# shubhamchandak94/HARC

Hardware: AMD Instinct MI355X
Metric: Mreads/s reorder+encode, 100 bp (higher is better)
Workload: dtype u64 (2-bit packed bases, XOR+popcount)

## Files before the change

### harc_amd/csrc/internal.h

```cpp
#pragma once
#include <hip/hip_runtime.h>
#include <stdint.h>
#include <stdio.h>
#include <string.h>
#include <map>
#include <string>
#include <utility>
#include <vector>
#include "../../include/harc_amd.h"

#define HARC_NONE 0xFFFFFFFFu
#define HARC_MAXW 8
#define HARC_MAXW3 12
#define HARC_MAXK (1u << 20)
#define HARC_LOOK_CHUNKS 16
#ifndef HARC_NSUGG
#define HARC_NSUGG 8
#endif

void harc_set_error(const char *fmt, ...);

#define HIP_TRY(expr)                                                                                          \
    do {                                                                                                       \
        hipError_t _e = (expr);                                                                                \
// ... 96 lines not shown
    harc_amd_counters C;
    uint64_t digest[4] = { 0, 0, 0, 0 }; bool have_digest = false;

    char *feed_ring = nullptr; size_t feed_ring_bytes = 0;

    void *d_tmp = nullptr; size_t tmp_bytes = 0;
};

struct HarcComm {
    int world = 1, rank = 0;
    virtual ~HarcComm() {}
    virtual int allgather_u64(harc_amd_ctx *c, const uint64_t *in, int n, uint64_t *out) = 0;
    virtual int alltoallv(harc_amd_ctx *c, int narr, const void *const *send, const size_t *const *soff, const size_t *const *sbytes,
                          void *const *recv, const size_t *const *roff, const size_t *const *rbytes) = 0;
    virtual int allreduce_min_u64(harc_amd_ctx *c, unsigned long long *d_buf, size_t n) = 0;
    virtual int wait(harc_amd_ctx *c, const char *what) = 0;
    virtual const char *name() const = 0;
};
int harc_in_reserve(harc_amd_ctx *c, harc_amd_ctx::InBuf *b, size_t bytes);
void harc_reset_shard(harc_amd_ctx *c);
void harc_drop_results(harc_amd_ctx *c);

int harc_dev_alloc(harc_amd_ctx *c, void **p, size_t bytes);
void harc_dev_free(harc_amd_ctx *c, void *p);
template <class T> static inline int dalloc(harc_amd_ctx *c, T **p, size_t n) { return harc_dev_alloc(c, (void **)p, n * sizeof(T) + 16); }
int harc_tmp_reserve(harc_amd_ctx *c, size_t bytes);
int harc_raw_alloc(harc_amd_ctx *c, void **p, size_t bytes);
void harc_raw_free(harc_amd_ctx *c, void *p);
typedef unsigned long long harc_mark_t;
harc_mark_t harc_pool_mark(harc_amd_ctx *c);
void harc_pool_release(harc_amd_ctx *c, harc_mark_t m);
struct PoolScope {
    harc_amd_ctx *c; harc_mark_t mk; bool armed = true;
    explicit PoolScope(harc_amd_ctx *c_) : c(c_), mk(harc_pool_mark(c_)) {}
    PoolScope(const PoolScope &) = delete;
    PoolScope &operator=(const PoolScope &) = delete;
    ~PoolScope() { if (armed) harc_pool_release(c, mk); }
    void keep() { armed = false; }
    void release_now() { if (armed) { harc_pool_release(c, mk); armed = false; } }
};

int prim_sort_pairs_u64_u32(harc_amd_ctx *c, const uint64_t *kin, uint64_t *kout, const uint32_t *vin, uint32_t *vout, size_t n, unsigned end_bit);
#define BL_TILE_WORDS 16384u
#define BL_PART_BITS 20
#define harc_bitmap_tiles(nwords) ((uint32_t)(((uint64_t)(nwords) + BL_TILE_WORDS - 1) / BL_TILE_WORDS))
#define harc_bitmap_item(w, b0, b1) (((uint64_t)((((uint32_t)(w) % BL_TILE_WORDS) << 10) | ((uint32_t)(b0) << 5) | (uint32_t)(b1)) << BL_PART_BITS) | (uint64_t)((uint32_t)(w) / BL_TILE_WORDS))
int harc_bitmap_from_items(harc_amd_ctx *c, const uint64_t *items, uint64_t *tmp, size_t n, uint64_t nwords, uint32_t *bitmap);
int prim_sort_keys_u64(harc_amd_ctx *c, const uint64_t *kin, uint64_t *kout, size_t n, unsigned end_bit);
int prim_excl_scan_u32(harc_amd_ctx *c, const uint32_t *in, uint32_t *out, size_t n);
int prim_excl_scan_u32_to_u64(harc_amd_ctx *c, const uint32_t *in, uint64_t *out, size_t n);
int prim_excl_scan_u8_to_u64(harc_amd_ctx *c, const uint8_t *in, uint64_t *out, size_t n);
int prim_incl_scan_u64(harc_amd_ctx *c, const uint64_t *in, uint64_t *out, size_t n);
int prim_incl_max_u32(harc_amd_ctx *c, const uint32_t *in, uint32_t *out, size_t n);
int prim_incl_max_u64(harc_amd_ctx *c, const uint64_t *in, uint64_t *out, size_t n);

int s1_pack_ascii(harc_amd_ctx *c, const char *d_ascii, uint32_t n, uint32_t stride, uint64_t *d_out);
int s1_pack3_ascii(harc_amd_ctx *c, const char *d_ascii, uint32_t n, uint32_t stride, uint64_t *d_out);
int s1_unpack_to_ascii(harc_amd_ctx *c, const uint64_t *d_reads, uint32_t n, char *d_out);
int s1_bucket_reads(harc_amd_ctx *c, const uint64_t *d_packed, uint32_t n, uint32_t nb, uint32_t *d_out);
int s1_partition_reads(harc_amd_ctx *c, const uint64_t *d_packed, uint32_t n, uint32_t nb, uint64_t *d_out, unsigned long long *d_counts);
int shard_partition(harc_amd_ctx *c, const uint64_t *d_words, uint32_t n, int nwords, bool three_bit, uint32_t nb, uint32_t gid0,
                    uint64_t *d_out, uint32_t *d_gid_out, unsigned long long *d_counts);
int shard_map_ids(harc_amd_ctx *c, uint32_t *d_v, uint64_t n, const uint32_t *d_map, uint32_t nmap, unsigned int *d_err);
int stage1_run(harc_amd_ctx *c);
int stage1_make_oriented(harc_amd_ctx *c, uint32_t i0 = 0, uint32_t i1 = 0xFFFFFFFFu);
int s1_orient(harc_amd_ctx *c, const uint64_t *reads, const uint32_t *order, const uint8_t *rc, uint32_t m, uint64_t *out);
int harc_dict_alloc(harc_amd_ctx *c, DictDev *d, uint32_t n, uint64_t cap_like);
int harc_dict_build(harc_amd_ctx *c, DictDev *d, uint64_t *keys, uint32_t *ids, uint32_t n, unsigned kbits);
void harc_dict_free(harc_amd_ctx *c, DictDev *d);
int stage2_run(harc_amd_ctx *c);
int pack_order_run(harc_amd_ctx *c);

static inline std::vector<uint8_t> &out_buf(harc_amd_ctx *c, int id, int shard) { harc_amd_ctx::OutBuf &o = c->out[std::make_pair(id, shard)]; o.ptr = nullptr; o.len = 0; return o.own; }
static inline void out_slice(harc_amd_ctx *c, int id, int shard, const void *p, size_t n) { harc_amd_ctx::OutBuf &o = c->out[std::make_pair(id, shard)]; o.own.clear(); o.ptr = (const uint8_t *)p; o.len = n; }
int harc_host_alloc(harc_amd_ctx *c, void **p, size_t bytes);
void harc_host_reset(harc_amd_ctx *c);
int harc_d2h(harc_amd_ctx *c, std::vector<uint8_t> &dst, const void *d_src, size_t bytes);

int build_line_index(harc_amd_ctx *c, const char *d_txt, uint64_t nbytes, const uint64_t **nls_out, uint64_t *total_lines_out);

struct BgzfCand { uint64_t off; uint32_t bsize, hdr, isize, crc; };
struct BgzfMember { uint64_t cdata, text; uint32_t clen, isize, crc, hdr; };
struct BgzfPlan { std::vector<BgzfMember> m; uint64_t text = 0, next = 0; };
int harc_bgzf_plan(harc_amd_ctx *c, const uint8_t *d_in, uint64_t n, uint64_t start, uint64_t own_end, uint64_t base_off, BgzfPlan *plan);
int harc_bgzf_run(harc_amd_ctx *c, const uint8_t *d_in, const BgzfPlan &plan, uint64_t base_off, char *d_out);

struct BgzfOutStats { uint64_t text = 0, bytes = 0, members = 0, stored = 0; double seconds = 0; };
int harc_bgzf_deflate(harc_amd_ctx *c, const char *d_text, uint64_t n_bytes, int32_t flags, uint8_t *d_out, uint64_t out_capacity, uint64_t *n_out, BgzfOutStats *st);
```

### harc_amd/csrc/prims.hip

```cpp
#include "devutil.h"
#include <rocprim/rocprim.hpp>

int harc_tmp_reserve(harc_amd_ctx *c, size_t bytes)
{
    if (bytes <= c->tmp_bytes) return HARC_AMD_OK;
    if (c->d_tmp) harc_raw_free(c, c->d_tmp);
    c->d_tmp = nullptr; c->tmp_bytes = 0;
    size_t want = bytes + (bytes >> 3) + 4096;
    RC_TRY(harc_raw_alloc(c, &c->d_tmp, want));
    c->tmp_bytes = want;
    return HARC_AMD_OK;
}

#define PRIM_CALL(call_with_tmp)                                \
    do {                                                        \
        size_t bytes = 0; void *tmp = nullptr;                  \
        HIP_TRY(call_with_tmp);                                 \
        RC_TRY(harc_tmp_reserve(c, bytes));                     \
        tmp = c->d_tmp; bytes = c->tmp_bytes;                   \
        HIP_TRY(call_with_tmp);                                 \
    } while (0)

int prim_sort_pairs_u64_u32(harc_amd_ctx *c, const uint64_t *kin, uint64_t *kout, const uint32_t *vin, uint32_t *vout, size_t n, unsigned end_bit)
{
    if (n == 0) return HARC_AMD_OK;
    if (end_bit > 64) end_bit = 64;
    PRIM_CALL(rocprim::radix_sort_pairs(tmp, bytes, kin, kout, vin, vout, n, 0u, end_bit, c->stream));
    return HARC_AMD_OK;
}

int prim_sort_keys_u64(harc_amd_ctx *c, const uint64_t *kin, uint64_t *kout, size_t n, unsigned end_bit)
{
    if (n == 0) return HARC_AMD_OK;
    if (end_bit > 64) end_bit = 64;
    if (end_bit < 1) end_bit = 1;
    PRIM_CALL(rocprim::radix_sort_keys(tmp, bytes, kin, kout, n, 0u, end_bit, c->stream));
    return HARC_AMD_OK;
}

int prim_excl_scan_u32(harc_amd_ctx *c, const uint32_t *in, uint32_t *out, size_t n)
{
    if (n == 0) return HARC_AMD_OK;
    PRIM_CALL(rocprim::exclusive_scan(tmp, bytes, in, out, 0u, n, rocprim::plus<uint32_t>(), c->stream));
    return HARC_AMD_OK;
}

struct u32_to_u64 { __host__ __device__ uint64_t operator()(uint32_t x) const { return (uint64_t)x; } };
struct u8_to_u64 { __host__ __device__ uint64_t operator()(uint8_t x) const { return (uint64_t)x; } };

int prim_excl_scan_u32_to_u64(harc_amd_ctx *c, const uint32_t *in, uint64_t *out, size_t n)
{
    if (n == 0) return HARC_AMD_OK;
    auto it = rocprim::make_transform_iterator(in, u32_to_u64());
    PRIM_CALL(rocprim::exclusive_scan(tmp, bytes, it, out, (uint64_t)0, n, rocprim::plus<uint64_t>(), c->stream));
    return HARC_AMD_OK;
}

int prim_excl_scan_u8_to_u64(harc_amd_ctx *c, const uint8_t *in, uint64_t *out, size_t n)
{
    if (n == 0) return HARC_AMD_OK;
    auto it = rocprim::make_transform_iterator(in, u8_to_u64());
    PRIM_CALL(rocprim::exclusive_scan(tmp, bytes, it, out, (uint64_t)0, n, rocprim::plus<uint64_t>(), c->stream));
    return HARC_AMD_OK;
}

int prim_incl_scan_u64(harc_amd_ctx *c, const uint64_t *in, uint64_t *out, size_t n)
{
    if (n == 0) return HARC_AMD_OK;
    PRIM_CALL(rocprim::inclusive_scan(tmp, bytes, in, out, n, rocprim::plus<uint64_t>(), c->stream));
    return HARC_AMD_OK;
}

int prim_incl_max_u32(harc_amd_ctx *c, const uint32_t *in, uint32_t *out, size_t n)
{
    if (n == 0) return HARC_AMD_OK;
    PRIM_CALL(rocprim::inclusive_scan(tmp, bytes, in, out, n, rocprim::maximum<uint32_t>(), c->stream));
    return HARC_AMD_OK;
}

int prim_incl_max_u64(harc_amd_ctx *c, const uint64_t *in, uint64_t *out, size_t n)
{
    if (n == 0) return HARC_AMD_OK;
    PRIM_CALL(rocprim::inclusive_scan(tmp, bytes, in, out, n, rocprim::maximum<uint64_t>(), c->stream));
    return HARC_AMD_OK;
}

__global__ void k_selftest_grid(uint64_t n, unsigned long long *out)
{
    const uint64_t i = harc_gid();
    unsigned long long one = i < n ? 1ULL : 0ULL, idx = i < n ? (unsigned long long)i : 0ULL;
    for (int o = 32; o > 0; o >>= 1) { one += __shfl_xor(one, o, 64); idx += __shfl_xor(idx, o, 64); }
    if ((threadIdx.x & 63) == 0 && one) { atomicAdd(&out[0], one); atomicAdd(&out[1], idx); }
}
__global__ void k_selftest_grid32(uint32_t n, unsigned long long *out)
{
    const uint32_t i = harc_gid32();
    unsigned long long one = i < n ? 1ULL : 0ULL, idx = i < n ? (unsigned long long)i : 0ULL;
    for (int o = 32; o > 0; o >>= 1) { one += __shfl_xor(one, o, 64); idx += __shfl_xor(idx, o, 64); }
    if ((threadIdx.x & 63) == 0 && one) { atomicAdd(&out[0], one); atomicAdd(&out[1], idx); }
}
__global__ void k_selftest_fold(uint64_t n, unsigned long long *out)
{
    const uint64_t wave = harc_bid() * 4 + (threadIdx.x >> 6);
    const int lane = threadIdx.x & 63;
    const uint64_t i = wave * 16 + (uint64_t)(lane >> 2);
    const bool mine = i < n && (lane & 3) == 0;
    unsigned long long one = mine ? 1ULL : 0ULL, idx = mine ? (unsigned long long)i : 0ULL;
    for (int o = 32; o > 0; o >>= 1) { one += __shfl_xor(one, o, 64); idx += __shfl_xor(idx, o, 64); }
    if (lane == 0 && one) { atomicAdd(&out[0], one); atomicAdd(&out[1], idx); }
}
extern "C" int harc_amd_selftest_launch(harc_amd_ctx *c, uint64_t n, uint64_t *visited, uint64_t *index_sum)
{
    if (!c || !visited || !index_sum) return HARC_AMD_EINVAL;
    HIP_TRY(hipSetDevice(c->P.device));
    unsigned long long *d = nullptr, h[6] = { 0, 0, 0, 0, 0, 0 };
    HIP_TRY(hipMalloc((void **)&d, sizeof h));
    const bool n32 = n <= 0xFFFFFFFFull;
    hipError_t e = hipMemsetAsync(d, 0, sizeof h, c->stream);
    if (e == hipSuccess) { hipLaunchKernelGGL(k_selftest_grid, harc_grid256(n), dim3(256), 0, c->stream, n, d); e = hipGetLastError(); }
    if (e == hipSuccess && n32) { hipLaunchKernelGGL(k_selftest_grid32, harc_grid256(n), dim3(256), 0, c->stream, (uint32_t)n, d + 2); e = hipGetLastError(); }
    if (e == hipSuccess) { hipLaunchKernelGGL(k_selftest_fold, harc_fold256((n + 63) / 64), dim3(256), 0, c->stream, n, d + 4); e = hipGetLastError(); }
    if (e == hipSuccess) e = hipMemcpyAsync(h, d, sizeof h, hipMemcpyDeviceToHost, c->stream);
    if (e == hipSuccess) e = hipStreamSynchronize(c->stream);
    (void)hipFree(d);
    if (e != hipSuccess) { harc_set_error("harc_amd_selftest_launch: %s", hipGetErrorString(e)); return HARC_AMD_ENODEVICE; }
    int k = 0;
    if (n32 && (h[2] != h[0] || h[3] != h[1])) k = 2;
    else if (h[4] != h[0] || h[5] != h[1]) k = 4;
    if (k) harc_set_error("harc_amd_selftest_launch: %s visited %llu items (index sum %llx), the thread-per-item grid %llu (%llx)", k == 2 ? "harc_gid32" : "harc_fold256 / harc_bid", h[k], h[k + 1], h[0], h[1]);
    *visited = h[k]; *index_sum = h[k + 1];
    return k ? HARC_AMD_EINTERNAL : HARC_AMD_OK;
}
```

### harc_amd/csrc/stage1.hip

```cpp
#include "devutil.h"
#include <stdlib.h>
#include <type_traits>

struct S1Args {
    int L, maxmatch, thresh, maxsearch, Lp;
    int ds[2], de[2], kbits[2];
    uint32_t N, K;
    const uint64_t *reads;
    HashSlot *slots[2];
    uint64_t cap[2];
    const uint32_t *ids[2];
    int firstmax;
    const uint32_t *bloom[2]; uint32_t bloom_lines; int bloom_nwin[2]; uint32_t bloom_mmask;
    const uint2 *largetab;
    uint64_t *mirror;
    unsigned long long *claimed;
    uint32_t *bid;
    ChainHdr *hdr;
    uint4 *cnt;
    uint2 *steps;
    uint8_t *need;
    uint32_t *seedbuf;
    uint32_t *needrank;
    uint32_t *rmeta;
    uint32_t own_mod, own_rem;
    uint32_t reseed_stress;
    uint32_t reseed_win;
    unsigned int *reseed_g;
    uint2 *cst2;
    uint32_t *bo;
    uint32_t *sugg;
    int S;
    int nsugg_per_seed;
    int nsugg_stride;
    uint2 *slog;
    uint2 *pg_rec;
    uint2 *pg_hdr;
    uint32_t *pg_cur;
    unsigned int *pg_count;
    long long *cursor;
    unsigned long long *coopcnt;
    unsigned long long *stats;
    const uint16_t *probe_tab;
    const uint32_t *lds_tab;
    int nprobe;
    int budget;
    int stepcap;
    int weedmin;
    int lazy;
    uint4 *cstat_coop;
    uint2 *csteps;
    uint4 *cstat;
    const uint2 *succ;
    unsigned long long *dbg;
// ... 156 lines not shown
    return HARC_AMD_OK;
}

template <int W> __global__ void k_keygen2(const uint64_t *reads, uint32_t n, int off0, int nbits0, int off1, int nbits1, uint64_t *keys0, uint64_t *keys1, uint32_t *ids)
{
    const uint32_t i = harc_gid32();
    if (i >= n) return;
    uint64_t r[W];
#pragma unroll
    for (int w = 0; w < W; w++) r[w] = reads[(size_t)i * W + w];
    {
        const int wi = off0 >> 6, sh = off0 & 63;
        const uint64_t lo = sel0<W>(r, wi), hi = sel0<W>(r, wi + 1);
        uint64_t v = sh ? ((lo >> sh) | (hi << (64 - sh))) : lo;
        if (nbits0 < 64) v &= ((uint64_t)1 << nbits0) - 1;
        keys0[i] = v;
    }
    {
        const int wi = off1 >> 6, sh = off1 & 63;
        const uint64_t lo = sel0<W>(r, wi), hi = sel0<W>(r, wi + 1);
        uint64_t v = sh ? ((lo >> sh) | (hi << (64 - sh))) : lo;
        if (nbits1 < 64) v &= ((uint64_t)1 << nbits1) - 1;
        keys1[i] = v;
    }
    ids[i] = i;
}
__global__ void k_large_sizes(const unsigned long long *list, uint32_t nlist, HashSlot *s0, HashSlot *s1, uint32_t *sz)
{
    const uint32_t b = harc_gid32();
    if (b >= nlist) return;
    const unsigned long long e = list[b];
    const HashSlot *slot = ((e & 1) ? s1 : s0) + (e >> 1);
    sz[b] = slot->count & SLOT_CNT_MASK;
}
template <int W> __global__ __launch_bounds__(64) void k_large_fill(const unsigned long long *list, uint32_t nlist, HashSlot *s0, HashSlot *s1, const uint32_t *ids0, const uint32_t *ids1,
                                                                   const uint64_t *moff, const uint64_t *reads, uint2 *largetab, uint64_t *mirror)
{
    const uint32_t b = blockIdx.y * gridDim.x + blockIdx.x;
    if (b >= nlist) return;
    const int lane = threadIdx.x;
    const unsigned long long e = list[b];
    const int l = (int)(e & 1);
    HashSlot *slot = (l ? s1 : s0) + (e >> 1);
    const uint32_t st = slot->start, cnt = slot->count & SLOT_CNT_MASK;
    const uint32_t *ids = (l ? ids1 : ids0) + st;
    const uint64_t m0 = moff[b];
    for (uint32_t k = lane; k < cnt; k += 64) {
        const uint32_t rid = ids[k];
#pragma unroll
        for (int w = 0; w < W; w++) mirror[(m0 + k) * W + w] = reads[(size_t)rid * W + w];
    }
    if (lane == 0) { largetab[b] = make_uint2(st, (uint32_t)m0); slot->start = b; }
}
__global__ void k_mark_heads(const uint64_t *skeys, uint32_t n, uint32_t *head)
{
    const uint32_t i = harc_gid32();
    if (i >= n) return;
    head[i] = (i == 0 || skeys[i] != skeys[i - 1]) ? 1u : 0u;
}
__global__ void k_bin_starts(const uint32_t *head, const uint32_t *binidx, uint32_t n, uint32_t *binstart, uint32_t *nbins, const uint64_t *skeys, uint64_t cap, uint64_t *v)
{
    const uint32_t i = harc_gid32();
    if (i >= n) return;
    if (head[i]) { const uint32_t b = binidx[i]; binstart[b] = i; v[b] = bucket_slot(skeys[i], cap) + (uint64_t)n - (uint64_t)b; }
    if (i == n - 1) *nbins = binidx[i] + head[i];
}
#define HARC_LARGEBIN 16u
#define HARC_STEP_CAP 12
#define HARC_BO_FREE 1u
#define HARC_BO_CAP 3u
#define HARC_SCAN_BUDGET 12
#define MIXED_MAX (1u << 20)
#define MIXED_BUDGET 200000u
__device__ __forceinline__ uint64_t rotl64(uint64_t x, unsigned r) { r &= 63u; return r ? (x << r) | (x >> (64u - r)) : x; }
__global__ void k_mixed_find(const uint64_t *rk, uint32_t n, unsigned sbits, uint64_t *sk, uint32_t *list, unsigned int *meta)
{
    const uint32_t i = harc_gid32();
    if (i >= n) return;
    const int shift = (int)(64u - sbits);
    const uint64_t b = rotl64(rk[i], 64u - sbits);
    sk[i] = b;
    if (i == 0) return;
    const uint64_t a = rotl64(rk[i - 1], 64u - sbits);
    if (a != b && (a >> shift) == (b >> shift)) { const unsigned int at = atomicAdd(&meta[0], 1u); if (at < MIXED_MAX) list[at] = i; else meta[1] = 1u; }
}
__global__ void k_mixed_own(const uint64_t *sk, int shift, uint32_t *list, unsigned int *meta)
{
    const uint32_t t = harc_gid32();
    const unsigned int nl = meta[0] < MIXED_MAX ? meta[0] : MIXED_MAX;
    if (t >= nl || meta[1]) return;
    const uint32_t i = list[t];
    const uint64_t top = sk[i] >> shift;
    for (uint32_t h = i; h > 0 && (sk[h - 1] >> shift) == top;) {
        h--;
        if (h > 0 && sk[h] != sk[h - 1] && (sk[h - 1] >> shift) == top) { list[t] = HARC_NONE; return; }
        if (i - h > MIXED_BUDGET) { meta[1] = 1u; return; }
    }
}
__global__ void k_mixed_fix(uint64_t *sk, uint32_t *ids, uint32_t n, int shift, const uint32_t *list, unsigned int *meta)
{
    const uint32_t t = harc_gid32();
    const unsigned int nl = meta[0] < MIXED_MAX ? meta[0] : MIXED_MAX;
    if (t >= nl || meta[1]) return;
    const uint32_t i = list[t];
    if (i == HARC_NONE) return;
    const uint64_t top = sk[i] >> shift;
    uint32_t h = i;
    while (h > 0 && (sk[h - 1] >> shift) == top) h--;
    uint32_t e = i + 1;
    while (e < n && (sk[e] >> shift) == top) { e++; if (e - h > MIXED_BUDGET) { meta[1] = 1u; return; } }
    uint32_t moves = 0;
    for (uint32_t x = h + 1; x < e; x++) {
        const uint64_t kx = sk[x]; const uint32_t vx = ids[x];
        uint32_t y = x;
        while (y > h && sk[y - 1] > kx) { sk[y] = sk[y - 1]; ids[y] = ids[y - 1]; y--; if (++moves > MIXED_BUDGET) { meta[1] = 1u; return; } }
        if (y != x) { sk[y] = kx; ids[y] = vx; }
    }
}
__global__ void k_scramble_keys(uint64_t *keys, uint32_t n, unsigned rot)
{
    const uint32_t i = harc_gid32();
    if (i < n) keys[i] = rotl64(key_scramble(keys[i]), rot);
}
__global__ void k_rotate_keys(uint64_t *keys, uint32_t n, unsigned rot)
{
    const uint32_t i = harc_gid32();
    if (i < n) keys[i] = rotl64(keys[i], rot);
}
#ifndef TP_SPAN
#define TP_SPAN 1280u
#endif
__global__ __launch_bounds__(256) void k_table_place(const uint64_t *skeys, const uint32_t *sids, const uint32_t *binstart, uint32_t nbins, uint32_t n, const uint64_t *q,
                              HashSlot *slots, uint64_t cap, uint32_t bigthresh,
                              unsigned long long *large_list, unsigned int *large_n, uint32_t large_max, uint32_t large_tag, uint32_t *nbins_p, int pass, uint32_t first_block, int fill)
{
    __shared__ uint4 tile[TP_SPAN];
    if (blockIdx.x < first_block) return;
    const uint32_t i = harc_gid32();
    const bool have = i < nbins;
    auto slot_of = [&](uint32_t k) -> uint64_t { return q[k] - (uint64_t)n + (uint64_t)k; };
    const uint32_t b0 = blockIdx.x * blockDim.x, b1 = b0 + blockDim.x < nbins ? b0 + blockDim.x : nbins;
    bool tiled = false; uint64_t lo = 0, hi = 0;
    if (pass == 0 && fill && b0 < nbins) {
        lo = b0 ? slot_of(b0 - 1) + 1 : 0;
        const uint64_t last = slot_of(b1 - 1);
        if (lo < cap) {
            hi = (last >= cap || b1 == nbins || slot_of(b1) >= cap) ? cap : last + 1;
            tiled = hi - lo <= TP_SPAN;
        }
    }
    if (tiled) {
        const uint4 z = make_uint4(0u, 0u, 0u, 0u);
        for (uint32_t j = threadIdx.x; j < (uint32_t)(hi - lo); j += blockDim.x) tile[j] = z;
        __syncthreads();
    }
    uint64_t sl = have ? slot_of(i) : 0;
    bool mine = have;
    if (mine && pass == 0 && sl >= cap && blockIdx.x + 64 < gridDim.x) { atomicAdd(nbins_p + 1, 1u); mine = false; }
    if (mine && (pass == 1) != (sl >= cap)) mine = false;
    if (mine) {
        const uint32_t st = binstart[i];
        const uint64_t key = skeys[st];
        uint32_t ovf = 0;
        if (pass == 0 && (sl & 3) == 0 && (uint64_t)i + 4 < (uint64_t)nbins) {
            const uint64_t s3 = slot_of(i + 3);
            if (s3 == sl + 3 && (bucket_slot(skeys[binstart[i + 4]], cap) >> 2) <= (sl >> 2)) ovf = SLOT_OVF;
        }
        if (pass == 0 && fill && !tiled) {
            const uint4 z = make_uint4(0u, 0u, 0u, 0u);
            for (uint64_t x = i ? slot_of(i - 1) + 1 : 0; x < sl; x++) *reinterpret_cast<uint4 *>(&slots[x]) = z;
            if (i + 1 == nbins || slot_of(i + 1) >= cap)
                for (uint64_t x = sl + 1; x < cap; x++) *reinterpret_cast<uint4 *>(&slots[x]) = z;
        }
        const uint32_t en = (i + 1 < nbins) ? binstart[i + 1] : n;
        const uint32_t cnt = en - st;
        if (cnt > SLOT_CNT_MASK) atomicAdd(nbins_p + 1, 1u);
        else {
            const unsigned long long meta = cnt == 1 ? ((unsigned long long)sids[st] | ((unsigned long long)(1u | SLOT_EMB) << 32))
                                                     : ((unsigned long long)st | ((unsigned long long)((cnt & SLOT_CNT_MASK) | ((bigthresh && cnt > bigthresh) ? SLOT_BIG : 0u)) << 32));
            if (pass == 1) {
                for (uint64_t bb = bucket_slot(key, cap) >> 2; bb < (cap >> 2); bb++) atomicOr(&slots[4 * bb].count, SLOT_OVF);
                sl = 0;
                for (;;) {
                    unsigned long long *mp = reinterpret_cast<unsigned long long *>(&slots[sl]) + 1;
                    if (atomicCAS(mp, 0ULL, meta) == 0ULL) break;
                    if ((sl & 3) == 3) atomicOr(&slots[sl - 3].count, SLOT_OVF);
                    if (++sl == cap) sl = 0;
                }
                slots[sl].key = key;
            } else {
                uint4 w; w.x = (uint32_t)key; w.y = (uint32_t)(key >> 32); w.z = (uint32_t)meta; w.w = (uint32_t)(meta >> 32) | ovf;
                if (tiled) tile[sl - lo] = w; else *reinterpret_cast<uint4 *>(&slots[sl]) = w;
            }
            if (large_list && cnt > HARC_LARGEBIN) {
                const unsigned int at = atomicAdd(large_n, 1u);
                if (at < large_max) large_list[at] = ((unsigned long long)sl << 1) | large_tag;
            }
        }
    }
    if (tiled) {
        __syncthreads();
        for (uint32_t j = threadIdx.x; j < (uint32_t)(hi - lo); j += blockDim.x) *reinterpret_cast<uint4 *>(&slots[lo + j]) = tile[j];
    }
}

__global__ void k_s1_bloom_keys(const uint64_t *keys, uint32_t n, uint32_t nlines, int nwin, uint32_t mmask, uint64_t *pk)
{
    const uint32_t i = harc_gid32();
    if (i >= n) return;
    uint32_t w, m;
    bloom_pos(keys[i], key_scramble(keys[i]), nlines, nwin, mmask, &w, &m);
    const uint32_t b0 = (uint32_t)__ffs((int)m) - 1u, b1 = 31u - (uint32_t)__clz((int)m);
    pk[i] = harc_bitmap_item(w, b0, b1);
}
__global__ __launch_bounds__(256) void k_s1_bloom_tile(const uint64_t *pk, uint32_t n, uint64_t nwords, uint32_t *bloom)
{
    __shared__ uint32_t tile[BL_TILE_WORDS];
    __shared__ uint32_t bounds[2];
    const uint32_t part = blockIdx.x;
// ... 1924 lines not shown
}
__global__ __launch_bounds__(256) void k_pages_out(const uint2 *pg_rec, const uint2 *pg_hdr, uint32_t npages, const uint32_t *n_main, const uint32_t *base_main,
                                                   uint32_t *order, uint8_t *flag, uint8_t *pos, uint8_t *rc)
{
    const uint32_t p = blockIdx.x * 4 + (threadIdx.x >> 6), lane = threadIdx.x & 63;
    if (p >= npages) return;
    const uint2 hd = pg_hdr[p];
    const uint32_t nm = n_main[hd.x], first = hd.y * 64u;
    if (first + lane >= nm) return;
    const uint2 r = pg_rec[(size_t)p * 64 + lane];
    const size_t at = (size_t)base_main[hd.x] + first + lane;
    order[at] = r.x; pos[at] = (uint8_t)(r.y & 0xFF);
    flag[at] = (r.y >> 8) & 1 ? '1' : '0'; rc[at] = (r.y >> 9) & 1 ? 'r' : 'd';
}
template <int W> __global__ void k_orient(const uint64_t *reads, const uint32_t *order, const uint8_t *rc, uint32_t m, int L, uint64_t *out)
{
    constexpr int RPW = 64 / W;
    const int lane = threadIdx.x & 63, rl = lane / W, w = lane % W;
    const uint64_t wave = harc_gid() >> 6;
    const uint64_t i64 = wave * RPW + (uint64_t)rl;
    const uint32_t i = (uint32_t)i64;
    const bool on = rl < RPW && i64 < m;
    uint64_t mine = 0; bool rev = false;
    if (on) {
        const uint32_t rid = order[i];
        mine = reads[(size_t)rid * W + w];
        rev = rc != nullptr && rc[i] == 'r';
    }
    uint64_t r[W], o[W];
#pragma unroll
    for (int k = 0; k < W; k++) r[k] = shfl_u64(mine, rl * W + k);
    if (!on) return;
    uint64_t ow = mine;
    if (rev) { rc_words<W>(r, L, o); ow = sel0<W>(o, w); }
    out[(size_t)i * W + w] = ow;
}

int harc_dict_alloc(harc_amd_ctx *c, DictDev *d, uint32_t n, uint64_t cap_like)
{
    d->cap = 0; d->slots = nullptr; d->ids = nullptr; d->d_nbins = nullptr;
    if (n == 0) return HARC_AMD_OK;
    if (cap_like) d->cap = cap_like;
    else {
        unsigned long long m = 4;
        size_t fr = 0, tot = 0;
        if (hipMemGetInfo(&fr, &tot) == hipSuccess) { fr += c->pool_total; while (m > 2 && ((double)m * n * sizeof(HashSlot) > 0.2 * (double)fr || (double)m * n * sizeof(HashSlot) > 0.15 * (double)tot)) m--; }
        if (c->P.table_slots_per_read >= 2 && c->P.table_slots_per_read <= 4) m = (unsigned long long)c->P.table_slots_per_read;
        if (const char *e = getenv("HARC_AMD_CAPMULT")) m = strtoull(e, nullptr, 10);
        d->cap = (((m < 2 ? 2 : m) * n + 4) + 3) & ~3ull;
    }
    RC_TRY(dalloc(c, &d->slots, d->cap)); RC_TRY(dalloc(c, &d->ids, n)); RC_TRY(dalloc(c, &d->d_nbins, 2));
    return HARC_AMD_OK;
}
int harc_dict_build(harc_amd_ctx *c, DictDev *d, uint64_t *keys, uint32_t *ids, uint32_t n, unsigned kbits)
{
    (void)kbits;
    if (n == 0) return HARC_AMD_OK;
    PoolScope scope(c);
    uint64_t *k1 = nullptr; uint32_t *h0 = nullptr, *b0 = nullptr, *bs = nullptr;
    RC_TRY(dalloc(c, &k1, n)); RC_TRY(dalloc(c, &h0, n)); RC_TRY(dalloc(c, &b0, n)); RC_TRY(dalloc(c, &bs, n));
    unsigned sbits = 64;
    { unsigned lg = 1; while (((uint64_t)1 << lg) < n) lg++; sbits = ((lg + 8 + 7) / 8) * 8; if (sbits > 64) sbits = 64; }
    if (const char *e = getenv("HARC_AMD_SORT_BITS")) { const int x = atoi(e); if (x >= 1 && x <= 64) sbits = (unsigned)x; }
    uint32_t *mixed = nullptr; unsigned int *mmeta = nullptr; uint64_t *k2 = nullptr;
    RC_TRY(dalloc(c, &mixed, MIXED_MAX)); RC_TRY(dalloc(c, &mmeta, 4));
    RC_TRY(dalloc(c, &k2, n));
    uint64_t *const k2v = k2;
    hipLaunchKernelGGL(k_scramble_keys, harc_grid256(n), dim3(256), 0, c->stream, keys, n, sbits < 64 ? sbits : 0u);
    uint32_t nbins = 0;
    for (;;) {
        HIP_TRY(hipMemsetAsync(mmeta, 0, 16, c->stream));
        HIP_TRY(hipMemsetAsync(d->d_nbins, 0, 8, c->stream));
        if (sbits < 64) {
            RC_TRY(prim_sort_pairs_u64_u32(c, keys, k2, ids, d->ids, n, sbits));
            hipLaunchKernelGGL(k_mixed_find, harc_grid256(n), dim3(256), 0, c->stream, (const uint64_t *)k2, n, sbits, k1, mixed, mmeta);
            hipLaunchKernelGGL(k_mixed_own, dim3(MIXED_MAX / 256), dim3(256), 0, c->stream, (const uint64_t *)k1, (int)(64 - sbits), mixed, mmeta);
            hipLaunchKernelGGL(k_mixed_fix, dim3(MIXED_MAX / 256), dim3(256), 0, c->stream, k1, d->ids, n, (int)(64 - sbits), (const uint32_t *)mixed, mmeta);
        } else RC_TRY(prim_sort_pairs_u64_u32(c, keys, k1, ids, d->ids, n, 64));
        hipLaunchKernelGGL(k_mark_heads, harc_grid256(n), dim3(256), 0, c->stream, k1, n, h0);
        RC_TRY(prim_excl_scan_u32(c, h0, b0, n));
        hipLaunchKernelGGL(k_bin_starts, harc_grid256(n), dim3(256), 0, c->stream, h0, b0, n, bs, d->d_nbins, (const uint64_t *)k1, d->cap, k2v);
        unsigned int mm[2] = { 0, 0 };
        HIP_TRY(hipMemcpyAsync(&nbins, d->d_nbins, 4, hipMemcpyDeviceToHost, c->stream));
        HIP_TRY(hipMemcpyAsync(mm, mmeta, 8, hipMemcpyDeviceToHost, c->stream));
        HIP_TRY(hipStreamSynchronize(c->stream));
        if (getenv("HARC_AMD_TRACE")) fprintf(stderr, "[index] sort on the top %u bits: %u places where different keys share them%s\n", sbits, mm[0], mm[1] ? " -- too many or too long, sorting on all bits" : "");
        if (!mm[1] || sbits == 64) break;
        hipLaunchKernelGGL(k_rotate_keys, harc_grid256(n), dim3(256), 0, c->stream, keys, n, 64u - sbits);
        sbits = 64;
    }
    const int fill = getenv("HARC_AMD_TABLE_FILL") ? atoi(getenv("HARC_AMD_TABLE_FILL")) != 0 : (uint64_t)nbins * 16 >= d->cap;
    if (!fill) HIP_TRY(hipMemsetAsync(d->slots, 0, d->cap * sizeof(HashSlot), c->stream));
    d->nbins = nbins;
    {
        uint64_t *v = k2v, *q = keys;
        const unsigned gb = (nbins + 255) / 256;
        RC_TRY(prim_incl_max_u64(c, v, q, nbins));
        for (int pass = 0; pass < 2; pass++)
            hipLaunchKernelGGL(k_table_place, dim3(gb), dim3(256), 0, c->stream, (const uint64_t *)k1, (const uint32_t *)d->ids, (const uint32_t *)bs, nbins, n, (const uint64_t *)q,
                               d->slots, d->cap, d->bigthresh, d->large_list, d->large_n, d->large_max, d->large_tag, d->d_nbins, pass, pass == 0 ? 0u : (gb > 64 ? gb - 64 : 0u), fill);
    }
    HIP_TRY(hipGetLastError());
    uint32_t nb2[2] = { 0, 0 };
    HIP_TRY(hipMemcpyAsync(nb2, d->d_nbins, 8, hipMemcpyDeviceToHost, c->stream));
    HIP_TRY(hipStreamSynchronize(c->stream));
    scope.release_now();
    if (nb2[1]) { harc_set_error("dictionary: %u bins hold more than %u reads with the same k-mer (count field of the slot), or lie more than 16384 bins beyond the end of the table", nb2[1], SLOT_CNT_MASK); return HARC_AMD_EINVAL; }
    return HARC_AMD_OK;
}
void harc_dict_free(harc_amd_ctx *c, DictDev *d)
{
    if (d->slots) harc_dev_free(c, d->slots);
    if (d->ids) harc_dev_free(c, d->ids);
    if (d->d_nbins) harc_dev_free(c, d->d_nbins);
    d->slots = nullptr; d->ids = nullptr; d->d_nbins = nullptr; d->cap = 0;
}

static std::vector<uint16_t> make_probe_table(const harc_amd_params &P)
{
    std::vector<uint16_t> t;
    for (int j = 0; j < P.maxmatch; j++) {
        for (int l = 0; l < 2; l++) if (P.dict_end[l] + j < P.readlen) t.push_back((uint16_t)(j | (0 << 8) | (l << 9)));
        for (int l = 0; l < 2; l++) if (P.dict_start[l] > j) t.push_back((uint16_t)(j | (1 << 8) | (l << 9)));
    }
    return t;
}

static uint32_t auto_chains(uint32_t N, int reads_per_chain)
{
    uint32_t k = N / (uint32_t)(reads_per_chain > 0 ? reads_per_chain : 2048);
    const uint32_t floor_k = N / 1024 < 2048 ? N / 1024 : 2048;
    if (k < floor_k) k = floor_k;
    if (k > 65536) k = 65536;
    if (k < 1) k = 1;
    return k;
}

struct EventRing {
    static constexpr int RING = 64;
    hipEvent_t ring[RING][2];
    int ring_used = 0; uint64_t ring_next = 0; double ms = 0; uint64_t launches = 0;
    EventRing() { for (int i = 0; i < RING; i++) ring[i][0] = ring[i][1] = nullptr; }
    ~EventRing() { for (int i = 0; i < ring_used; i++) { (void)hipEventDestroy(ring[i][0]); (void)hipEventDestroy(ring[i][1]); } }
    int next_pair(hipEvent_t **pair)
    {
        const int k = (int)(ring_next % RING);
        if (k >= ring_used) { HIP_TRY(hipEventCreate(&ring[k][0])); HIP_TRY(hipEventCreate(&ring[k][1])); ring_used = k + 1; }
        else RC_TRY(collect(k));
        ring_next++; launches++;
        *pair = ring[k];
        return HARC_AMD_OK;
    }
    int collect(int k) { float x = 0; HIP_TRY(hipEventSynchronize(ring[k][1])); HIP_TRY(hipEventElapsedTime(&x, ring[k][0], ring[k][1])); ms += x; return HARC_AMD_OK; }
    int collect_all() { const uint64_t n = ring_next < (uint64_t)RING ? ring_next : (uint64_t)RING; for (uint64_t i = 0; i < n; i++) RC_TRY(collect((int)i)); ring_next = 0; return HARC_AMD_OK; }
};
struct S1Resources {
    hipEvent_t e[3] = { nullptr, nullptr, nullptr };
    hipEvent_t eb[2] = { nullptr, nullptr };
    EventRing dense, coop;
    unsigned long long *h_stats = nullptr;
// ... 491 lines not shown
```

Before: 696.1.

## Fuse bin-head marking, bin scan and slot max-scan into one custom-operator scan

The separate head-marking kernel, exclusive scan, bin-start kernel and max-scan over slot positions are replaced with a single rocprim inclusive scan. It uses a custom associative operator that carries a bin count and a running max, and writes bin starts and slot positions through a custom output iterator. Sorted keys also stay in rotated form, and consumers unrotate them on the fly, which drops the rotated-copy buffer and extra passes. An optional host verification path, enabled by an environment variable, checks the placement against a sequential reference. The cost is a heavier scan element (16 bytes), more complex iterator logic, and the rotate arithmetic in the mixed-fix and placement kernels.

```diff
diff --git a/harc_amd/csrc/dict_place.h b/harc_amd/csrc/dict_place.h
--- /dev/null
+++ b/harc_amd/csrc/dict_place.h
@@ -0,0 +1,87 @@
+#pragma once
+#include <stddef.h>
+#include <stdint.h>
+#include <vector>
+#if defined(__HIPCC__)
+#define DP_HD __host__ __device__ __forceinline__
+#define DP_HDM __host__ __device__ __forceinline__
+#else
+#define DP_HD static inline
+#define DP_HDM inline
+#endif
+
+#define DP_NONE (-((int64_t)1 << 62))
+struct DpAcc {
+    uint32_t c;
+    uint32_t head;
+    int64_t m;
+};
+struct DpCombine {
+    DP_HDM DpAcc operator()(const DpAcc &a, const DpAcc &b) const
+    {
+        DpAcc r;
+        r.c = a.c + b.c;
+        r.head = b.head;
+        const int64_t mb = b.m - (int64_t)a.c;
+        r.m = a.m > mb ? a.m : mb;
+        return r;
+    }
+};
+DP_HD uint64_t dp_unrot(uint64_t x, unsigned rot) { rot &= 63u; return rot ? (x >> rot) | (x << (64u - rot)) : x; }
+DP_HD uint64_t dp_home(uint64_t h, uint64_t cap)
+{
+    const uint64_t nb = cap >> 2;
+#if defined(__HIP_DEVICE_COMPILE__)
+    if (nb >> 32) return __umul64hi(h, nb) << 2;
+#else
+    if (nb >> 32) return (uint64_t)(((unsigned __int128)h * nb) >> 64) << 2;
+#endif
+    return (((h >> 32) * nb) >> 32) << 2;
+}
+DP_HD DpAcc dp_element(uint64_t key_rot, uint64_t prev_rot, bool first, unsigned rot, uint64_t cap)
+{
+    DpAcc e;
+    if (first || key_rot != prev_rot) { e.c = 1; e.head = 1; e.m = (int64_t)dp_home(dp_unrot(key_rot, rot), cap); }
+    else { e.c = 0; e.head = 0; e.m = DP_NONE; }
+    return e;
+}
+DP_HD uint64_t dp_q(int64_t m, uint32_t n) { return (uint64_t)(m + (int64_t)n); }
+
+static inline long long dict_place_reference(const uint64_t *keys, const uint32_t *ids, uint32_t n, uint64_t cap, uint32_t bigthresh,
+                                             uint32_t emb, uint32_t big, uint32_t ovf, uint32_t cnt_mask, std::vector<uint32_t> &slots,
+                                             std::vector<uint64_t> *wrapped_slots = nullptr)
+{
+    slots.assign((size_t)cap * 4, 0u);
+    if (wrapped_slots) wrapped_slots->clear();
+    uint64_t prev = 0; bool any = false, wrapped = false;
+    long long nbins = 0;
+    for (uint32_t st = 0; st < n;) {
+        uint32_t en = st + 1;
+        while (en < n && keys[en] == keys[st]) en++;
+        const uint32_t cnt = en - st;
+        if (cnt > cnt_mask) return -1;
+        const uint64_t key = keys[st], home = dp_home(key, cap);
+        uint64_t sl = (any && prev + 1 > home) ? prev + 1 : home;
+        if (sl >= cap || wrapped) {
+            for (uint64_t b = home >> 2; b < (cap >> 2); b++) slots[(size_t)b * 16 + 3] |= ovf;
+            uint64_t x = 0;
+            while (slots[(size_t)x * 4 + 3] & ~ovf) {
+                if ((x & 3) == 3) slots[(size_t)(x - 3) * 4 + 3] |= ovf;
+                if (++x == cap) return -1;
+            }
+            sl = x; wrapped = true;
+            if (wrapped_slots) wrapped_slots->push_back(sl);
+        } else {
+            for (uint64_t b = home >> 2; b < (sl >> 2); b++) slots[(size_t)b * 16 + 3] |= ovf;
+            prev = sl;
+        }
+        any = true;
+        uint32_t *s = &slots[(size_t)sl * 4];
+        s[0] = (uint32_t)key; s[1] = (uint32_t)(key >> 32);
+        if (cnt == 1) { s[2] = ids[st]; s[3] |= 1u | emb; }
+        else { s[2] = st; s[3] |= cnt | ((bigthresh && cnt > bigthresh) ? big : 0u); }
+        nbins++;
+        st = en;
+    }
+    return nbins;
+}
diff --git a/harc_amd/csrc/internal.h b/harc_amd/csrc/internal.h
--- a/harc_amd/csrc/internal.h
+++ b/harc_amd/csrc/internal.h
@@ -172,7 +172,7 @@
 int prim_excl_scan_u8_to_u64(harc_amd_ctx *c, const uint8_t *in, uint64_t *out, size_t n);
 int prim_incl_scan_u64(harc_amd_ctx *c, const uint64_t *in, uint64_t *out, size_t n);
 int prim_incl_max_u32(harc_amd_ctx *c, const uint32_t *in, uint32_t *out, size_t n);
-int prim_incl_max_u64(harc_amd_ctx *c, const uint64_t *in, uint64_t *out, size_t n);
+int prim_bins_from_sorted_keys(harc_amd_ctx *c, const uint64_t *keys_rot, uint32_t n, unsigned rot, uint64_t cap, uint32_t *binstart, uint64_t *q, uint32_t *d_nbins);
 
 int s1_pack_ascii(harc_amd_ctx *c, const char *d_ascii, uint32_t n, uint32_t stride, uint64_t *d_out);
 int s1_pack3_ascii(harc_amd_ctx *c, const char *d_ascii, uint32_t n, uint32_t stride, uint64_t *d_out);
diff --git a/harc_amd/csrc/prims.hip b/harc_amd/csrc/prims.hip
--- a/harc_amd/csrc/prims.hip
+++ b/harc_amd/csrc/prims.hip
@@ -1,5 +1,7 @@
 #include "devutil.h"
+#include "dict_place.h"
 #include <rocprim/rocprim.hpp>
+#include <iterator>
 
 int harc_tmp_reserve(harc_amd_ctx *c, size_t bytes)
 {
@@ -78,10 +80,43 @@
     return HARC_AMD_OK;
 }
 
-int prim_incl_max_u64(harc_amd_ctx *c, const uint64_t *in, uint64_t *out, size_t n)
+struct DpInput {
+    const uint64_t *keys; uint32_t n; unsigned rot; uint64_t cap;
+    __host__ __device__ DpAcc operator()(uint32_t i) const
+    {
+        if (i >= n) { DpAcc e; e.c = 0; e.head = 0; e.m = DP_NONE; return e; }
+        return dp_element(keys[i], i ? keys[i - 1] : 0, i == 0, rot, cap);
+    }
+};
+struct DpStore {
+    uint32_t *binstart; uint64_t *q; uint32_t *nbins; uint32_t n, i;
+    __host__ __device__ const DpStore &operator=(const DpAcc &a) const
+    {
+        if (a.head) { binstart[a.c - 1] = i; q[a.c - 1] = dp_q(a.m, n); }
+        if (i == n - 1) *nbins = a.c;
+        return *this;
+    }
+};
+struct DpOutput {
+    using iterator_category = std::random_access_iterator_tag;
+    using value_type = DpAcc;
+    using difference_type = std::ptrdiff_t;
+    using pointer = void;
+    using reference = DpStore;
+    uint32_t *binstart; uint64_t *q; uint32_t *nbins; uint32_t n; size_t at;
+    __host__ __device__ DpStore operator[](size_t d) const { return DpStore{ binstart, q, nbins, n, (uint32_t)(at + d) }; }
+    __host__ __device__ DpStore operator*() const { return (*this)[0]; }
+    __host__ __device__ DpOutput operator+(size_t d) const { DpOutput o = *this; o.at += d; return o; }
+    __host__ __device__ DpOutput &operator+=(size_t d) { at += d; return *this; }
+    __host__ __device__ DpOutput &operator++() { at++; return *this; }
+};
+using DpScanConfig = rocprim::scan_config<256, 8, rocprim::block_load_method::block_load_transpose, rocprim::block_store_method::block_store_transpose, rocprim::block_scan_algorithm::using_warp_scan>;
+int prim_bins_from_sorted_keys(harc_amd_ctx *c, const uint64_t *keys_rot, uint32_t n, unsigned rot, uint64_t cap, uint32_t *binstart, uint64_t *q, uint32_t *d_nbins)
 {
     if (n == 0) return HARC_AMD_OK;
-    PRIM_CALL(rocprim::inclusive_scan(tmp, bytes, in, out, n, rocprim::maximum<uint64_t>(), c->stream));
+    auto in = rocprim::make_transform_iterator(rocprim::make_counting_iterator<uint32_t>(0u), DpInput{ keys_rot, n, rot, cap });
+    DpOutput out{ binstart, q, d_nbins, n, 0 };
+    PRIM_CALL(rocprim::inclusive_scan<DpScanConfig>(tmp, bytes, in, out, (size_t)n, DpCombine(), c->stream));
     return HARC_AMD_OK;
 }
 
diff --git a/harc_amd/csrc/stage1.hip b/harc_amd/csrc/stage1.hip
--- a/harc_amd/csrc/stage1.hip
+++ b/harc_amd/csrc/stage1.hip
@@ -1,5 +1,8 @@
 #include "devutil.h"
+#include "dict_place.h"
 #include <stdlib.h>
+#include <algorithm>
+#include <array>
 #include <type_traits>
 
 struct S1Args {
@@ -262,19 +265,6 @@
     }
     if (lane == 0) { largetab[b] = make_uint2(st, (uint32_t)m0); slot->start = b; }
 }
-__global__ void k_mark_heads(const uint64_t *skeys, uint32_t n, uint32_t *head)
-{
-    const uint32_t i = harc_gid32();
-    if (i >= n) return;
-    head[i] = (i == 0 || skeys[i] != skeys[i - 1]) ? 1u : 0u;
-}
-__global__ void k_bin_starts(const uint32_t *head, const uint32_t *binidx, uint32_t n, uint32_t *binstart, uint32_t *nbins, const uint64_t *skeys, uint64_t cap, uint64_t *v)
-{
-    const uint32_t i = harc_gid32();
-    if (i >= n) return;
-    if (head[i]) { const uint32_t b = binidx[i]; binstart[b] = i; v[b] = bucket_slot(skeys[i], cap) + (uint64_t)n - (uint64_t)b; }
-    if (i == n - 1) *nbins = binidx[i] + head[i];
-}
 #define HARC_LARGEBIN 16u
 #define HARC_STEP_CAP 12
 #define HARC_BO_FREE 1u
@@ -283,48 +273,47 @@
 #define MIXED_MAX (1u << 20)
 #define MIXED_BUDGET 200000u
 __device__ __forceinline__ uint64_t rotl64(uint64_t x, unsigned r) { r &= 63u; return r ? (x << r) | (x >> (64u - r)) : x; }
-__global__ void k_mixed_find(const uint64_t *rk, uint32_t n, unsigned sbits, uint64_t *sk, uint32_t *list, unsigned int *meta)
+__global__ void k_mixed_find(const uint64_t *rk, uint32_t n, unsigned sbits, uint32_t *list, unsigned int *meta)
 {
     const uint32_t i = harc_gid32();
-    if (i >= n) return;
+    if (i >= n || i == 0) return;
     const int shift = (int)(64u - sbits);
-    const uint64_t b = rotl64(rk[i], 64u - sbits);
-    sk[i] = b;
-    if (i == 0) return;
-    const uint64_t a = rotl64(rk[i - 1], 64u - sbits);
+    const uint64_t b = dp_unrot(rk[i], sbits), a = dp_unrot(rk[i - 1], sbits);
     if (a != b && (a >> shift) == (b >> shift)) { const unsigned int at = atomicAdd(&meta[0], 1u); if (at < MIXED_MAX) list[at] = i; else meta[1] = 1u; }
 }
-__global__ void k_mixed_own(const uint64_t *sk, int shift, uint32_t *list, unsigned int *meta)
+__global__ void k_mixed_own(const uint64_t *rk, unsigned rot, int shift, uint32_t *list, unsigned int *meta)
 {
     const uint32_t t = harc_gid32();
     const unsigned int nl = meta[0] < MIXED_MAX ? meta[0] : MIXED_MAX;
     if (t >= nl || meta[1]) return;
+    auto sk = [&](uint32_t x) -> uint64_t { return dp_unrot(rk[x], rot); };
     const uint32_t i = list[t];
-    const uint64_t top = sk[i] >> shift;
-    for (uint32_t h = i; h > 0 && (sk[h - 1] >> shift) == top;) {
+    const uint64_t top = sk(i) >> shift;
+    for (uint32_t h = i; h > 0 && (sk(h - 1) >> shift) == top;) {
         h--;
-        if (h > 0 && sk[h] != sk[h - 1] && (sk[h - 1] >> shift) == top) { list[t] = HARC_NONE; return; }
+        if (h > 0 && sk(h) != sk(h - 1) && (sk(h - 1) >> shift) == top) { list[t] = HARC_NONE; return; }
         if (i - h > MIXED_BUDGET) { meta[1] = 1u; return; }
     }
 }
-__global__ void k_mixed_fix(uint64_t *sk, uint32_t *ids, uint32_t n, int shift, const uint32_t *list, unsigned int *meta)
+__global__ void k_mixed_fix(uint64_t *rk, unsigned rot, uint32_t *ids, uint32_t n, int shift, const uint32_t *list, unsigned int *meta)
 {
     const uint32_t t = harc_gid32();
     const unsigned int nl = meta[0] < MIXED_MAX ? meta[0] : MIXED_MAX;
     if (t >= nl || meta[1]) return;
+    auto sk = [&](uint32_t x) -> uint64_t { return dp_unrot(rk[x], rot); };
     const uint32_t i = list[t];
     if (i == HARC_NONE) return;
-    const uint64_t top = sk[i] >> shift;
+    const uint64_t top = sk(i) >> shift;
     uint32_t h = i;
-    while (h > 0 && (sk[h - 1] >> shift) == top) h--;
+    while (h > 0 && (sk(h - 1) >> shift) == top) h--;
     uint32_t e = i + 1;
-    while (e < n && (sk[e] >> shift) == top) { e++; if (e - h > MIXED_BUDGET) { meta[1] = 1u; return; } }
+    while (e < n && (sk(e) >> shift) == top) { e++; if (e - h > MIXED_BUDGET) { meta[1] = 1u; return; } }
     uint32_t moves = 0;
     for (uint32_t x = h + 1; x < e; x++) {
-        const uint64_t kx = sk[x]; const uint32_t vx = ids[x];
+        const uint64_t rx = rk[x], kx = dp_unrot(rx, rot); const uint32_t vx = ids[x];
         uint32_t y = x;
-        while (y > h && sk[y - 1] > kx) { sk[y] = sk[y - 1]; ids[y] = ids[y - 1]; y--; if (++moves > MIXED_BUDGET) { meta[1] = 1u; return; } }
-        if (y != x) { sk[y] = kx; ids[y] = vx; }
+        while (y > h && sk(y - 1) > kx) { rk[y] = rk[y - 1]; ids[y] = ids[y - 1]; y--; if (++moves > MIXED_BUDGET) { meta[1] = 1u; return; } }
+        if (y != x) { rk[y] = rx; ids[y] = vx; }
     }
 }
 __global__ void k_scramble_keys(uint64_t *keys, uint32_t n, unsigned rot)
@@ -342,7 +331,7 @@
 #endif
 __global__ __launch_bounds__(256) void k_table_place(const uint64_t *skeys, const uint32_t *sids, const uint32_t *binstart, uint32_t nbins, uint32_t n, const uint64_t *q,
                               HashSlot *slots, uint64_t cap, uint32_t bigthresh,
-                              unsigned long long *large_list, unsigned int *large_n, uint32_t large_max, uint32_t large_tag, uint32_t *nbins_p, int pass, uint32_t first_block, int fill)
+                              unsigned long long *large_list, unsigned int *large_n, uint32_t large_max, uint32_t large_tag, uint32_t *nbins_p, int pass, uint32_t first_block, int fill, unsigned rot)
 {
     __shared__ uint4 tile[TP_SPAN];
     if (blockIdx.x < first_block) return;
@@ -370,11 +359,11 @@
     if (mine && (pass == 1) != (sl >= cap)) mine = false;
     if (mine) {
         const uint32_t st = binstart[i];
-        const uint64_t key = skeys[st];
+        const uint64_t key = dp_unrot(skeys[st], rot);
         uint32_t ovf = 0;
         if (pass == 0 && (sl & 3) == 0 && (uint64_t)i + 4 < (uint64_t)nbins) {
             const uint64_t s3 = slot_of(i + 3);
-            if (s3 == sl + 3 && (bucket_slot(skeys[binstart[i + 4]], cap) >> 2) <= (sl >> 2)) ovf = SLOT_OVF;
+            if (s3 == sl + 3 && (bucket_slot(dp_unrot(skeys[binstart[i + 4]], rot), cap) >> 2) <= (sl >> 2)) ovf = SLOT_OVF;
         }
         if (pass == 0 && fill && !tiled) {
             const uint4 z = make_uint4(0u, 0u, 0u, 0u);
@@ -2405,34 +2394,60 @@
     RC_TRY(dalloc(c, &d->slots, d->cap)); RC_TRY(dalloc(c, &d->ids, n)); RC_TRY(dalloc(c, &d->d_nbins, 2));
     return HARC_AMD_OK;
 }
+#define INDEX_VERIFY_MAX (1u << 24)
+static int dict_verify(harc_amd_ctx *c, const DictDev *d, const uint64_t *skeys_rot, unsigned rot, uint32_t n, uint32_t nbins)
+{
+    if (n > INDEX_VERIFY_MAX) { harc_set_error("HARC_AMD_INDEX_VERIFY: %u keys, the host check takes at most %u", n, INDEX_VERIFY_MAX); return HARC_AMD_EINVAL; }
+    std::vector<uint64_t> hk(n), wrapped; std::vector<uint32_t> hi(n), got((size_t)d->cap * 4), want;
+    HIP_TRY(hipMemcpyAsync(hk.data(), skeys_rot, (size_t)n * 8, hipMemcpyDeviceToHost, c->stream));
+    HIP_TRY(hipMemcpyAsync(hi.data(), d->ids, (size_t)n * 4, hipMemcpyDeviceToHost, c->stream));
+    HIP_TRY(hipMemcpyAsync(got.data(), d->slots, (size_t)d->cap * 16, hipMemcpyDeviceToHost, c->stream));
+    HIP_TRY(hipStreamSynchronize(c->stream));
+    for (uint32_t i = 0; i < n; i++) hk[i] = dp_unrot(hk[i], rot);
+    for (uint32_t i = 1; i < n; i++)
+        if (hk[i] < hk[i - 1] || (hk[i] == hk[i - 1] && hi[i] < hi[i - 1])) { harc_set_error("index verify: keys / ids out of order at %u of %u", i, n); return HARC_AMD_EINTERNAL; }
+    const long long nb = dict_place_reference(hk.data(), hi.data(), n, d->cap, d->bigthresh, SLOT_EMB, SLOT_BIG, SLOT_OVF, SLOT_CNT_MASK, want, &wrapped);
+    if (nb != (long long)nbins) { harc_set_error("index verify: %u bins, the sequential placement makes %lld", nbins, nb); return HARC_AMD_EINTERNAL; }
+    if (wrapped.size() > 1) {
+        std::vector<std::array<uint32_t, 4>> a, b;
+        for (uint64_t sl : wrapped) {
+            uint32_t *g = &got[(size_t)sl * 4], *w = &want[(size_t)sl * 4];
+            a.push_back({ g[0], g[1], g[2], g[3] & ~SLOT_OVF }); b.push_back({ w[0], w[1], w[2], w[3] & ~SLOT_OVF });
+        }
+        std::sort(a.begin(), a.end()); std::sort(b.begin(), b.end());
+        if (a != b) { harc_set_error("index verify: the %zu bins that wrap around the end of the table differ from the sequential placement", wrapped.size()); return HARC_AMD_EINTERNAL; }
+        for (uint64_t sl : wrapped) for (int w = 0; w < 4; w++) got[(size_t)sl * 4 + w] = (got[(size_t)sl * 4 + w] & (w == 3 ? SLOT_OVF : 0u)) | (want[(size_t)sl * 4 + w] & (w == 3 ? ~SLOT_OVF : ~0u));
+    }
+    for (size_t x = 0; x < got.size(); x++)
+        if (got[x] != want[x]) { harc_set_error("index verify: slot %zu word %zu is %08x, the sequential placement has %08x (%u keys, %u bins, %llu slots)", x / 4, x % 4, got[x], want[x], n, nbins, (unsigned long long)d->cap); return HARC_AMD_EINTERNAL; }
+    if (getenv("HARC_AMD_TRACE")) fprintf(stderr, "[index] verified: %u keys, %u bins, %llu slots, %zu bins wrapped\n", n, nbins, (unsigned long long)d->cap, wrapped.size());
+    return HARC_AMD_OK;
+}
 int harc_dict_build(harc_amd_ctx *c, DictDev *d, uint64_t *keys, uint32_t *ids, uint32_t n, unsigned kbits)
 {
     (void)kbits;
     if (n == 0) return HARC_AMD_OK;
     PoolScope scope(c);
-    uint64_t *k1 = nullptr; uint32_t *h0 = nullptr, *b0 = nullptr, *bs = nullptr;
-    RC_TRY(dalloc(c, &k1, n)); RC_TRY(dalloc(c, &h0, n)); RC_TRY(dalloc(c, &b0, n)); RC_TRY(dalloc(c, &bs, n));
     unsigned sbits = 64;
     { unsigned lg = 1; while (((uint64_t)1 << lg) < n) lg++; sbits = ((lg + 8 + 7) / 8) * 8; if (sbits > 64) sbits = 64; }
     if (const char *e = getenv("HARC_AMD_SORT_BITS")) { const int x = atoi(e); if (x >= 1 && x <= 64) sbits = (unsigned)x; }
-    uint32_t *mixed = nullptr; unsigned int *mmeta = nullptr; uint64_t *k2 = nullptr;
+    uint32_t *mixed = nullptr, *bs = nullptr; unsigned int *mmeta = nullptr; uint64_t *sk = nullptr, *q = nullptr;
     RC_TRY(dalloc(c, &mixed, MIXED_MAX)); RC_TRY(dalloc(c, &mmeta, 4));
-    RC_TRY(dalloc(c, &k2, n));
-    uint64_t *const k2v = k2;
+    RC_TRY(dalloc(c, &sk, n));
+    RC_TRY(dalloc(c, &bs, n)); RC_TRY(dalloc(c, &q, n));
     hipLaunchKernelGGL(k_scramble_keys, harc_grid256(n), dim3(256), 0, c->stream, keys, n, sbits < 64 ? sbits : 0u);
-    uint32_t nbins = 0;
+    uint32_t nbins = 0; unsigned rot = 0;
     for (;;) {
         HIP_TRY(hipMemsetAsync(mmeta, 0, 16, c->stream));
         HIP_TRY(hipMemsetAsync(d->d_nbins, 0, 8, c->stream));
+        rot = sbits < 64 ? sbits : 0u;
+        RC_TRY(prim_sort_pairs_u64_u32(c, keys, sk, ids, d->ids, n, sbits));
         if (sbits < 64) {
-            RC_TRY(prim_sort_pairs_u64_u32(c, keys, k2, ids, d->ids, n, sbits));
-            hipLaunchKernelGGL(k_mixed_find, harc_grid256(n), dim3(256), 0, c->stream, (const uint64_t *)k2, n, sbits, k1, mixed, mmeta);
-            hipLaunchKernelGGL(k_mixed_own, dim3(MIXED_MAX / 256), dim3(256), 0, c->stream, (const uint64_t *)k1, (int)(64 - sbits), mixed, mmeta);
-            hipLaunchKernelGGL(k_mixed_fix, dim3(MIXED_MAX / 256), dim3(256), 0, c->stream, k1, d->ids, n, (int)(64 - sbits), (const uint32_t *)mixed, mmeta);
-        } else RC_TRY(prim_sort_pairs_u64_u32(c, keys, k1, ids, d->ids, n, 64));
-        hipLaunchKernelGGL(k_mark_heads, harc_grid256(n), dim3(256), 0, c->stream, k1, n, h0);
-        RC_TRY(prim_excl_scan_u32(c, h0, b0, n));
-        hipLaunchKernelGGL(k_bin_starts, harc_grid256(n), dim3(256), 0, c->stream, h0, b0, n, bs, d->d_nbins, (const uint64_t *)k1, d->cap, k2v);
+            hipLaunchKernelGGL(k_mixed_find, harc_grid256(n), dim3(256), 0, c->stream, (const uint64_t *)sk, n, sbits, mixed, mmeta);
+            hipLaunchKernelGGL(k_mixed_own, dim3(MIXED_MAX / 256), dim3(256), 0, c->stream, (const uint64_t *)sk, rot, (int)(64 - sbits), mixed, mmeta);
+            hipLaunchKernelGGL(k_mixed_fix, dim3(MIXED_MAX / 256), dim3(256), 0, c->stream, sk, rot, d->ids, n, (int)(64 - sbits), (const uint32_t *)mixed, mmeta);
+        }
+        RC_TRY(prim_bins_from_sorted_keys(c, sk, n, rot, d->cap, bs, q, d->d_nbins));
         unsigned int mm[2] = { 0, 0 };
         HIP_TRY(hipMemcpyAsync(&nbins, d->d_nbins, 4, hipMemcpyDeviceToHost, c->stream));
         HIP_TRY(hipMemcpyAsync(mm, mmeta, 8, hipMemcpyDeviceToHost, c->stream));
@@ -2446,19 +2461,18 @@
     if (!fill) HIP_TRY(hipMemsetAsync(d->slots, 0, d->cap * sizeof(HashSlot), c->stream));
     d->nbins = nbins;
     {
-        uint64_t *v = k2v, *q = keys;
         const unsigned gb = (nbins + 255) / 256;
-        RC_TRY(prim_incl_max_u64(c, v, q, nbins));
         for (int pass = 0; pass < 2; pass++)
-            hipLaunchKernelGGL(k_table_place, dim3(gb), dim3(256), 0, c->stream, (const uint64_t *)k1, (const uint32_t *)d->ids, (const uint32_t *)bs, nbins, n, (const uint64_t *)q,
-                               d->slots, d->cap, d->bigthresh, d->large_list, d->large_n, d->large_max, d->large_tag, d->d_nbins, pass, pass == 0 ? 0u : (gb > 64 ? gb - 64 : 0u), fill);
+            hipLaunchKernelGGL(k_table_place, dim3(gb), dim3(256), 0, c->stream, (const uint64_t *)sk, (const uint32_t *)d->ids, (const uint32_t *)bs, nbins, n, (const uint64_t *)q,
+                               d->slots, d->cap, d->bigthresh, d->large_list, d->large_n, d->large_max, d->large_tag, d->d_nbins, pass, pass == 0 ? 0u : (gb > 64 ? gb - 64 : 0u), fill, rot);
     }
     HIP_TRY(hipGetLastError());
     uint32_t nb2[2] = { 0, 0 };
     HIP_TRY(hipMemcpyAsync(nb2, d->d_nbins, 8, hipMemcpyDeviceToHost, c->stream));
     HIP_TRY(hipStreamSynchronize(c->stream));
+    if (nb2[1]) { harc_set_error("dictionary: %u bins hold more than %u reads with the same k-mer (count field of the slot), or lie more than 16384 bins beyond the end of the table", nb2[1], SLOT_CNT_MASK); return HARC_AMD_EINVAL; }
+    if (const char *e = getenv("HARC_AMD_INDEX_VERIFY")) if (atoi(e)) RC_TRY(dict_verify(c, d, sk, rot, n, nbins));
     scope.release_now();
-    if (nb2[1]) { harc_set_error("dictionary: %u bins hold more than %u reads with the same k-mer (count field of the slot), or lie more than 16384 bins beyond the end of the table", nb2[1], SLOT_CNT_MASK); return HARC_AMD_EINVAL; }
     return HARC_AMD_OK;
 }
 void harc_dict_free(harc_amd_ctx *c, DictDev *d)
```

After: 697.5 (median of 6 runs). No clear change (+0.2%).
